# bxlab/bx-python

Hardware: AMD Instinct MI355X
Metric: M overlap-queries/s at 100M x 10M intervals (count-only) (higher is better)
Workload: dtype int32

## Files before the change

### bx-python_amd/csrc/common.hpp

```cpp
#pragma once
#include <hip/hip_runtime.h>

#include <cstdarg>
#include <cstdint>
#include <cstdio>
#include <cstring>
#include <string>

#include "../../include/bxmi.h"

namespace bxmi {

std::string &last_error();
int fail(int code, const char *fmt, ...);

#define BXMI_HIP(expr)                                                                          \
    do {                                                                                        \
        hipError_t _e = (expr);                                                                 \
        if (_e != hipSuccess)                                                                   \
            return ::bxmi::fail(_e == hipErrorOutOfMemory ? BXMI_ENOMEM : BXMI_EHIP, "%s: %s (%s:%d)", #expr, \
                                hipGetErrorString(_e), __FILE__, __LINE__);                     \
    } while (0)

#define BXMI_TRY(expr)            \
// ... 27 lines not shown
        hipError_t e = hipMalloc(&np, want);
        if (e != hipSuccess) return fail(BXMI_ENOMEM, "hipMalloc(%zu): %s", want, hipGetErrorString(e));
        if (keep && p && cap) {
            e = hipMemcpyAsync(np, p, cap, hipMemcpyDeviceToDevice, st);
            if (e == hipSuccess) e = hipStreamSynchronize(st);
            if (e != hipSuccess) {
                (void)hipFree(np);
                return fail(BXMI_EHIP, "grow copy: %s", hipGetErrorString(e));
            }
        }
        if (p) (void)hipFree(p);
        p = np;
        cap = want;
        return BXMI_OK;
    }
    template <typename T>
    T *as() const
    {
        return reinterpret_cast<T *>(p);
    }
};

struct DeviceProps {
    int cus = 256;
    int device = -1;
};
const DeviceProps &device_props();

inline int stream_grid(int64_t work_items, int items_per_block)
{
    int64_t need = (work_items + items_per_block - 1) / items_per_block;
    int64_t cap = (int64_t)device_props().cus * 8;
    int64_t g = need < cap ? need : cap;
    if (g < 1) g = 1;
    return (int)g;
}

inline int64_t div_up(int64_t a, int64_t b) { return (a + b - 1) / b; }

#define BXMI_WAVE 64

#define BX_GLOBAL __attribute__((address_space(1)))
template <typename T>
__device__ __forceinline__ T BX_GLOBAL *as_global(T *p)
{
    return (T BX_GLOBAL *)p;
}
typedef int bx_v4i __attribute__((ext_vector_type(4)));
__device__ __forceinline__ int4 load_int4(const int32_t BX_GLOBAL *p)
{
    const bx_v4i v = *reinterpret_cast<const bx_v4i BX_GLOBAL *>(p);
    return make_int4(v.x, v.y, v.z, v.w);
}
__device__ __forceinline__ void store_int4(int32_t BX_GLOBAL *p, int a, int b, int c, int d)
{
    *reinterpret_cast<bx_v4i BX_GLOBAL *>(p) = bx_v4i{a, b, c, d};
}

__device__ __forceinline__ int lane_id() { return (int)(threadIdx.x & 63); }

#define BXMI_DPP_QUAD_XOR1 0xB1
#define BXMI_DPP_QUAD_XOR2 0x4E
#define BXMI_DPP_HALF_MIRROR 0x141

__device__ __forceinline__ int group8_sum_dpp(int v)
{
    v += __builtin_amdgcn_update_dpp(0, v, BXMI_DPP_QUAD_XOR1, 0xf, 0xf, false);
    v += __builtin_amdgcn_update_dpp(0, v, BXMI_DPP_QUAD_XOR2, 0xf, 0xf, false);
    v += __builtin_amdgcn_update_dpp(0, v, BXMI_DPP_HALF_MIRROR, 0xf, 0xf, false);
    return v;
}

__device__ __forceinline__ int group8_sum_shfl(int v)
{
    v += __shfl_xor(v, 1, 64);
    v += __shfl_xor(v, 2, 64);
    v += __shfl_xor(v, 4, 64);
    return v;
}

__device__ __forceinline__ long long wave_sum_i64(long long v)
{
#pragma unroll
    for (int off = 32; off > 0; off >>= 1) v += __shfl_down(v, off, 64);
    return v;
}

__device__ __forceinline__ unsigned long long lanemask_lt()
{
    return (1ull << lane_id()) - 1ull;
}

__device__ __forceinline__ void block_accumulate_i64(long long v, long long *red, unsigned long long *global_acc)
{
    v = wave_sum_i64(v);
    int w = threadIdx.x >> 6;
    if (lane_id() == 0) red[w] = v;
    __syncthreads();
    if (threadIdx.x == 0) {
        long long s = 0;
        int nw = (blockDim.x + 63) >> 6;
        for (int i = 0; i < nw; i++) s += red[i];
        if (s) atomicAdd(global_acc, (unsigned long long)s);
    }
}

// ... 11 lines not shown
```

### bx-python_amd/csrc/count_bitmap.hpp

```cpp
#pragma once

namespace bxmi {

constexpr int BM_NB = PT_NB;
constexpr unsigned BM_REC_ESC = 0xFFFFFFFFu;
constexpr int BM_MIN_SHIFT = 5;
constexpr int BM_GROUP_TILES = 64;
constexpr int BM_CHUNK = 65536;
constexpr int BM_HARD = 127;
constexpr int BM_LONG_CAP = 480;

struct BmGeom {
    int32_t cmin;
    int32_t cmax;
    int32_t shift;
    int32_t nce;
    int32_t ncs;
    int32_t stride;
    int32_t f;
    int32_t rshift;
    int32_t dshift;
};

__device__ __forceinline__ unsigned bm_len_esc(const BmGeom &g) { return (1u << (32 - g.rshift)) - 1u; }
// ... 159 lines not shown
    return descent;
}

__device__ __forceinline__ void bm_bounds_outer(const int32_t *__restrict__ qs, int64_t nq, const BmBounds &B)
{
    const int first = bm_bounds_upto(B, qs[0]), last = bm_bounds_upto(B, qs[nq - 1]);
    for (int u = 0; u < first; u++) B.bounds[u] = 0u;
    for (int u = last; u <= B.units; u++) B.bounds[u] = (unsigned)nq;
}

template <bool BOUNDS>
__global__ __launch_bounds__(256) void bm_sorted_check_kernel(const int32_t *__restrict__ qs, int64_t nq, unsigned *__restrict__ unsorted, BmBounds B)
{
    if (BOUNDS && blockIdx.x == 0 && threadIdx.x == 0) bm_bounds_outer(qs, nq, B);
    for (int64_t c = blockIdx.x; c * BM_CHECK_CH < nq; c += gridDim.x) {
        if (__hip_atomic_load(unsorted, __ATOMIC_RELAXED, __HIP_MEMORY_SCOPE_WORKGROUP) != 0) return;
        const bool descent = bm_check_chunk<BOUNDS>(qs, nq, c, B);
        if (__syncthreads_or(descent)) {
            if (threadIdx.x == 0) __hip_atomic_store(unsorted, 1u, __ATOMIC_RELAXED, __HIP_MEMORY_SCOPE_WORKGROUP);
            return;
        }
    }
}

__device__ __forceinline__ unsigned bm_bucket_of(int qs, const BmGeom &g)
{
    if (qs < g.cmin) return 0;
    const unsigned b = ((unsigned)qs - (unsigned)g.cmin) >> g.shift;
    return b < (unsigned)(BM_NB - 1) ? b : (unsigned)(BM_NB - 1);
}

template <int SUB>
__device__ __forceinline__ unsigned bm_sort_key_of(int qs, const BmGeom &g)
{
    if (SUB == 1) return bm_bucket_of(qs, g);
    if (qs < g.cmin) return 0;
    const unsigned b = ((unsigned)qs - (unsigned)g.cmin) >> (g.shift - 1);
    return b < (unsigned)(2 * BM_NB - 1) ? b : (unsigned)(2 * BM_NB - 1);
}

__device__ __forceinline__ unsigned bm_record_of(int qs, int qe, const BmGeom &g)
{
    const unsigned rel = (unsigned)qs - (unsigned)g.cmin;
    const unsigned len = (unsigned)qe - (unsigned)qs;
    const bool ok = qs >= g.cmin && (rel >> g.shift) < (unsigned)BM_NB && qe > qs && len < bm_len_esc(g);
    return ok ? ((rel & ((1u << (g.shift + g.f)) - 1u)) | (len << g.rshift)) : BM_REC_ESC;
}

constexpr int BM_PAD_ROOM = 4096 + 544;
#ifndef BM_TS_EXP
#define BM_TS_EXP 0
#endif

template <int THREADS, int ITEMS, bool PAD = false, int SUB = 1, bool TOT = false>
__global__ __launch_bounds__(THREADS) void bm_tile_sort_kernel(const BmSeg *__restrict__ segs, const unsigned short *__restrict__ tile_seg,
                                                               unsigned *__restrict__ recs ,
                                                               unsigned short *__restrict__ slots ,
                                                               unsigned short *__restrict__ tbl ,
                                                               const unsigned *__restrict__ gate ,
                                                               unsigned *__restrict__ tend ,
                                                               unsigned short *__restrict__ tbl2 ,
                                                               const BmSegChunk par, const int npar , const BmParOut po,
                                                               unsigned *__restrict__ tesc = nullptr )
{
    constexpr int TILE = THREADS * ITEMS;
    if (gate && *gate == 0) return;
    static_assert(!TOT || (PAD && SUB == 1), "total-only batches: the persistent walk on padded runs");
    constexpr int NBK = BM_NB * SUB;
    constexpr int BPT = NBK / THREADS;
    static_assert(NBK % THREADS == 0 && (BPT == 2 || BPT == 4), "2 or 4 buckets per thread");
    static_assert(SUB == 1 || (SUB == 2 && !PAD && BPT == 4), "half buckets: packed runs, 1024-thread shapes");
    constexpr int STAGED = PAD ? TILE + 3 * THREADS : TILE;
    constexpr int STRIDE = PAD ? TILE + BM_PAD_ROOM : TILE;
    extern __shared__ __attribute__((aligned(16))) int32_t dyn[];
    unsigned *staged = reinterpret_cast<unsigned *>(dyn);
    unsigned *cnt = staged + STAGED;
    unsigned short *toff = reinterpret_cast<unsigned short *>(cnt + NBK);
    unsigned *scan_tmp = reinterpret_cast<unsigned *>(toff + NBK);
    const int64_t tile = blockIdx.x;
    BmGeom g;
    const int32_t BX_GLOBAL *__restrict__ qs, *__restrict__ qe;
    int64_t nq, ltile, ntiles_seg;
    if (npar) {
        if (blockIdx.x == 0) bm_write_params(par, npar, po);
        int i = 0;
        while (i + 1 < npar && tile >= par.seg[i].tile_end) i++;
        g = par.seg[i].g;
        ltile = tile - par.seg[i].tile0, ntiles_seg = par.seg[i].ntiles;
        qs = as_global(par.seg[i].qs) + ltile * TILE, qe = as_global(par.seg[i].qe) + ltile * TILE;
        nq = par.seg[i].nq - ltile * TILE;
    } else {
        const BmSeg &sg = segs[tile_seg[tile]];
        g = sg.g;
        ltile = tile - sg.tile0, ntiles_seg = sg.ntiles;
        qs = as_global(sg.qs) + ltile * TILE, qe = as_global(sg.qe) + ltile * TILE;
        nq = sg.nq - ltile * TILE;
    }
    if (ltile >= ntiles_seg) return;
    recs += tile * STRIDE, slots += tile * TILE;
    const int64_t base = 0;
    const int n = (int)(nq < TILE ? nq : TILE);
    int n_out = n;
    for (int i = threadIdx.x; i < NBK; i += THREADS) cnt[i] = 0;
    __syncthreads();
    unsigned br[ITEMS];
    int4 vs[ITEMS / 4], ve[ITEMS / 4];
    if (n == TILE) {
#pragma unroll
        for (int j = 0; j < ITEMS / 4; j++) vs[j] = load_int4(qs + base + 4 * (j * THREADS + (int)threadIdx.x));
#pragma unroll
        for (int j = 0; j < ITEMS / 4; j++) ve[j] = load_int4(qe + base + 4 * (j * THREADS + (int)threadIdx.x));
#pragma unroll
        for (int j = 0; j < ITEMS / 4; j++) {
            const unsigned bx = bm_sort_key_of<SUB>(vs[j].x, g), by = bm_sort_key_of<SUB>(vs[j].y, g), bz = bm_sort_key_of<SUB>(vs[j].z, g),
                           bw = bm_sort_key_of<SUB>(vs[j].w, g);
            const unsigned b0 = (unsigned)__builtin_amdgcn_readfirstlane((int)bx);
            if (__all(bx == b0 && by == b0 && bz == b0 && bw == b0)) {
                unsigned r0 = 0;
                if (lane_id() == 0) r0 = atomicAdd(&cnt[b0], 256u);
                r0 = (unsigned)__builtin_amdgcn_readfirstlane((int)r0) + 4u * (unsigned)lane_id();
                br[4 * j + 0] = (b0 << 16) | (r0 + 0);
                br[4 * j + 1] = (b0 << 16) | (r0 + 1);
                br[4 * j + 2] = (b0 << 16) | (r0 + 2);
                br[4 * j + 3] = (b0 << 16) | (r0 + 3);
            } else {
                if (BM_TS_EXP == 1) {
                    const unsigned fake = 4u * (unsigned)(j * THREADS + (int)threadIdx.x);
                    br[4 * j + 0] = (bx << 16) | (fake + 0u), br[4 * j + 1] = (by << 16) | (fake + 1u);
                    br[4 * j + 2] = (bz << 16) | (fake + 2u), br[4 * j + 3] = (bw << 16) | (fake + 3u);
                } else {
                br[4 * j + 0] = (bx << 16) | atomicAdd(&cnt[bx], 1u);
                br[4 * j + 1] = (by << 16) | atomicAdd(&cnt[by], 1u);
                br[4 * j + 2] = (bz << 16) | atomicAdd(&cnt[bz], 1u);
                br[4 * j + 3] = (bw << 16) | atomicAdd(&cnt[bw], 1u);
                }
            }
        }
    } else {
#pragma unroll
        for (int j = 0; j < ITEMS; j++) {
            const int k = j * THREADS + threadIdx.x;
            if (k < n) {
                const unsigned b = bm_sort_key_of<SUB>(qs[base + k], g);
                br[j] = (b << 16) | atomicAdd(&cnt[b], 1u);
            }
        }
    }
    __syncthreads();
    {
        unsigned c[BPT], sum = 0;
#pragma unroll
        for (int u = 0; u < BPT; u++) {
            c[u] = cnt[BPT * threadIdx.x + u];
            sum += c[u];
        }
        unsigned tot;
        unsigned exc;
        if (PAD) {
            const int lane = lane_id();
            const int lanes = (1 << g.f) / BPT;
            unsigned usum = sum;
            for (int d = 1; d < lanes; d <<= 1) usum += (unsigned)__shfl_xor((int)usum, d, 64);
            const unsigned padded = (usum + 3u) & ~3u;
            const bool leader = (lane & (lanes - 1)) == 0;
            const unsigned before = block_exclusive_scan(leader ? padded : 0u, OpSum(), 0u, scan_tmp, &tot);
            const unsigned ubase = (unsigned)__shfl((int)before, lane & ~(lanes - 1), 64);
            unsigned inc = sum;
            for (int d = 1; d < lanes; d <<= 1) {
                const unsigned up = (unsigned)__shfl_up((int)inc, d, 64);
                if ((lane & (lanes - 1)) >= d) inc += up;
            }
            exc = ubase + inc - sum;
            if (leader)
                for (unsigned k = usum; k < padded; k++) staged[ubase + k] = BM_REC_ESC;
            n_out = BM_TS_EXP == 1 ? n : (int)tot;
            if (threadIdx.x == 0) tend[tile] = tot;
        } else {
            exc = block_exclusive_scan(sum, OpSum(), 0u, scan_tmp, &tot);
        }
        unsigned short o[BPT];
#pragma unroll
        for (int u = 0; u < BPT; u++) {
            o[u] = (unsigned short)exc;
            toff[BPT * threadIdx.x + u] = o[u];
            exc += c[u];
        }
        if (SUB == 2) {
            *reinterpret_cast<unsigned *>(tbl + tile * BM_NB + 2 * threadIdx.x) = (unsigned)o[0] | ((unsigned)o[2 % BPT] << 16);
            *reinterpret_cast<uint2 *>(tbl2 + tile * NBK + BPT * threadIdx.x) =
                make_uint2((unsigned)o[0] | ((unsigned)o[1] << 16), (unsigned)o[2 % BPT] | ((unsigned)o[BPT - 1] << 16));
        } else {
        unsigned short *row = tbl + tile * BM_NB + BPT * threadIdx.x;
        if (BPT == 4)
            *reinterpret_cast<uint2 *>(row) = make_uint2((unsigned)o[0] | ((unsigned)o[1] << 16), (unsigned)o[2] | ((unsigned)o[BPT - 1] << 16));
        else
            *reinterpret_cast<unsigned *>(row) = (unsigned)o[0] | ((unsigned)o[1] << 16);
        }
    }
    __syncthreads();
    bool esc = false;
    if (n == TILE) {
        uint2 *l4 = reinterpret_cast<uint2 *>(slots + base);
#pragma unroll
        for (int j = 0; j < ITEMS / 4; j++) {
            const unsigned s0 = toff[br[4 * j + 0] >> 16] + (br[4 * j + 0] & 0xffffu), s1 = toff[br[4 * j + 1] >> 16] + (br[4 * j + 1] & 0xffffu);
            const unsigned s2 = toff[br[4 * j + 2] >> 16] + (br[4 * j + 2] & 0xffffu), s3 = toff[br[4 * j + 3] >> 16] + (br[4 * j + 3] & 0xffffu);
            if (BM_TS_EXP == 3) {
                if ((s0 ^ s1 ^ s2 ^ s3 ^ (unsigned)vs[j].x ^ (unsigned)ve[j].y) == 0x9e3779b9u) staged[0] = s0;
                continue;
            }
            const unsigned r0 = bm_record_of(vs[j].x, ve[j].x, g), r1 = bm_record_of(vs[j].y, ve[j].y, g);
            const unsigned r2 = bm_record_of(vs[j].z, ve[j].z, g), r3 = bm_record_of(vs[j].w, ve[j].w, g);
            staged[s0] = r0, staged[s1] = r1, staged[s2] = r2, staged[s3] = r3;
            if (TOT)
                esc |= r0 == BM_REC_ESC || r1 == BM_REC_ESC || r2 == BM_REC_ESC || r3 == BM_REC_ESC;
            else
                l4[j * THREADS + threadIdx.x] = make_uint2(s0 | (s1 << 16), s2 | (s3 << 16));
        }
    } else {
#pragma unroll
        for (int j = 0; j < ITEMS; j++) {
            const int k = j * THREADS + threadIdx.x;
            if (k < n) {
                const unsigned s = toff[br[j] >> 16] + (br[j] & 0xffffu);
                const unsigned r = bm_record_of(qs[base + k], qe[base + k], g);
                staged[s] = r;
                if (TOT)
                    esc |= r == BM_REC_ESC;
                else
                    slots[base + k] = (unsigned short)s;
            }
        }
    }
    if (TOT) {
        const int any = __syncthreads_or(esc ? 1 : 0);
        if (threadIdx.x == 0) tesc[tile] = (unsigned)(any != 0);
    } else {
        __syncthreads();
    }
    int4 *out = reinterpret_cast<int4 *>(recs + base);
    const int n4 = BM_TS_EXP == 2 ? 0 : (n_out + 3) >> 2;
    for (int i = threadIdx.x; i < n4; i += THREADS) out[i] = reinterpret_cast<const int4 *>(staged)[i];
}


template <int NBK = BM_NB>
__global__ __launch_bounds__(256) void bm_transpose_kernel(const unsigned short *__restrict__ tbl, const BmSeg *__restrict__ segs,
                                                           const unsigned short *__restrict__ tile_seg, int tile_log2,
                                                           unsigned *__restrict__ runT , int64_t ntp,
                                                           unsigned *__restrict__ grpcnt , const unsigned *__restrict__ gate)
{
    __shared__ unsigned short t[BM_GROUP_TILES][66];
    if (gate && *gate == 0) return;
    const int grp = blockIdx.x, b0 = blockIdx.y * 64;
    {
        const int r = threadIdx.x >> 2, q = threadIdx.x & 3;
        const int64_t tile = (int64_t)grp * BM_GROUP_TILES + r;
        const BmSeg &sg = segs[tile_seg[tile]];
        const bool live = tile - sg.tile0 < sg.ntiles;
        const int64_t left = sg.nq - ((tile - sg.tile0) << tile_log2);
        const unsigned ntile = !live ? 0u : (left < ((int64_t)1 << tile_log2) ? (unsigned)left : 1u << tile_log2);
        const unsigned short *row = tbl + tile * NBK + b0 + 16 * q;
        uint4 a = make_uint4(0, 0, 0, 0), c = a;
        if (live) {
            a = *reinterpret_cast<const uint4 *>(row);
            c = *reinterpret_cast<const uint4 *>(row + 8);
        }
        const unsigned w[8] = {a.x, a.y, a.z, a.w, c.x, c.y, c.z, c.w};
#pragma unroll
        for (int i = 0; i < 8; i++) {
            t[r][16 * q + 2 * i] = (unsigned short)(w[i] & 0xffffu);
            t[r][16 * q + 2 * i + 1] = (unsigned short)(w[i] >> 16);
        }
        if (q == 3) t[r][64] = (unsigned short)(b0 + 64 < NBK ? (live ? row[16] : 0) : ntile);
    }
    __syncthreads();
    {
        const int c = threadIdx.x >> 2, q = threadIdx.x & 3;
        unsigned *dst = runT + (int64_t)(b0 + c) * ntp + (int64_t)grp * BM_GROUP_TILES + 16 * q;
        unsigned sum = 0;
        unsigned v[16];
#pragma unroll
        for (int i = 0; i < 16; i++) {
            const unsigned off = t[16 * q + i][c], len = (unsigned)(unsigned short)(t[16 * q + i][c + 1] - t[16 * q + i][c]);
            v[i] = off | (len << 16);
            sum += len;
        }
#pragma unroll
        for (int i = 0; i < 4; i++) reinterpret_cast<uint4 *>(dst)[i] = make_uint4(v[4 * i], v[4 * i + 1], v[4 * i + 2], v[4 * i + 3]);
        sum += __shfl_xor(sum, 1, 64);
        sum += __shfl_xor(sum, 2, 64);
        if (q == 0 && grpcnt) grpcnt[(int64_t)grp * NBK + b0 + c] = sum;
    }
}

constexpr int BM_PLAN_BATCH = 16;
template <bool EMIT, int UNITS>
// ... 363 lines not shown
```

### bx-python_amd/csrc/intervals.hip

```cpp
#include <climits>
#include <vector>
#include <algorithm>
#include <atomic>
#include <condition_variable>
#include <mutex>
#include <thread>
#include <utility>

#include "primitives.hpp"
#include "count_plan.hpp"

#include "count_direct.hpp"
#include "count_parts.hpp"
#include "count_bitmap.hpp"
#include "count_slices.hpp"
#include "find_exchange.hpp"
#include "count_dense.hpp"
#include "find_sorted.hpp"
#include "find_direct.hpp"
#include "find_neighbors.hpp"
#include "cluster.hpp"

namespace bxmi {

static int64_t g_opt_partition = -1;
constexpr int64_t g_opt_partition_min = 4 << 20;
constexpr int PT_MAX_SUB = 1;
constexpr int PT_SLOT_STRIDE = PT_SLOTS + 8;
static int64_t g_opt_sorted_path = 1;
static int64_t g_opt_bitmap = -1;
static int64_t g_opt_bitmap_min = 2 << 20;
static int64_t g_opt_bm_variant = -1;
static int64_t g_opt_fx_direct = -1;
static int64_t g_opt_find_sliced = 1;
static int64_t g_opt_slice = -1;
static int64_t g_opt_sl_f = -1;
constexpr int64_t g_opt_bm_chunk = 0;
static int64_t g_opt_sl_run_cap = 160;
static int64_t g_opt_sl_flat = 1;
constexpr int64_t g_opt_sl_rbits = 20;
static int64_t g_opt_sl_lanes = 0;
static int64_t g_opt_bm_hard_ppm = 2000;
static int64_t g_opt_flat = -1;
static int64_t g_opt_sparse = -1;
static int64_t g_opt_bo_cell_log2 = 0;
constexpr int64_t g_opt_bo_min_per_unit = 4096;
static int64_t g_opt_sorted_cells = 1;
static int64_t g_opt_dense = -1;
static int64_t g_opt_bd_chunk = 0;
static int64_t g_opt_bd_table_from = 0;
static int64_t g_opt_bd_blocks = 0;
static int64_t g_opt_bd_w8 = -1;
static int64_t g_opt_order_skip = -1;
static int64_t g_opt_clumped = -1;
static int64_t g_opt_tot_walk = 1;
static int64_t g_opt_host_chunk = 8 << 20;
static int64_t g_opt_host_touchers = 2;
constexpr int64_t g_opt_bd_unit_log2 = 0;

struct IvlOpt {
    const char *key;
    int64_t *var;
    int64_t (*norm)(int64_t);
};
static const IvlOpt IVL_OPTS[] = {
    {"ivl.partition", &g_opt_partition, nullptr},
    {"ivl.sorted_path", &g_opt_sorted_path, [](int64_t value) -> int64_t { return value != 0; }},
    {"ivl.bitmap_min", &g_opt_bitmap_min, nullptr},
    {"ivl.bitmap", &g_opt_bitmap, nullptr},
    {"ivl.bm_variant", &g_opt_bm_variant, [](int64_t value) -> int64_t { return value < 0 || value > 2 ? -1 : value; }},
    {"ivl.find_sliced", &g_opt_find_sliced, [](int64_t value) -> int64_t { return value != 0; }},
    {"ivl.fx_direct", &g_opt_fx_direct, [](int64_t value) -> int64_t { return value < 0 ? -1 : value != 0; }},
    {"ivl.slice", &g_opt_slice, nullptr},
    {"ivl.sl_f", &g_opt_sl_f, [](int64_t value) -> int64_t { return value > SL_MAX_F ? SL_MAX_F : value; }},
    {"ivl.sl_run_cap", &g_opt_sl_run_cap, [](int64_t value) -> int64_t { return value < 8 ? 8 : value; }},
    {"ivl.sl_flat", &g_opt_sl_flat, [](int64_t value) -> int64_t { return value != 0; }},
    {"ivl.sl_lanes", &g_opt_sl_lanes, [](int64_t value) -> int64_t { return value == 16 || value == 64 ? value : (value == 1 ? -1 : 0);  }},
    {"ivl.bm_hard_ppm", &g_opt_bm_hard_ppm, nullptr},
    {"ivl.flat", &g_opt_flat, nullptr},
    {"ivl.dense", &g_opt_dense, nullptr},
    {"ivl.sparse", &g_opt_sparse, nullptr},
    {"ivl.sorted_cells", &g_opt_sorted_cells, [](int64_t value) -> int64_t { return value != 0; }},
    {"ivl.bo_cell_log2", &g_opt_bo_cell_log2, [](int64_t value) -> int64_t { return value < BO_MIN_K || value > BO_MAX_K ? 0 : value; }},
    {"ivl.bd_chunk", &g_opt_bd_chunk, [](int64_t value) -> int64_t { return value < 0 ? 0 : value; }},
    {"ivl.bd_blocks", &g_opt_bd_blocks, [](int64_t value) -> int64_t { return value != 0; }},
    {"ivl.bd_table_from", &g_opt_bd_table_from, [](int64_t value) -> int64_t { return value < 1 || value > 64 ? 0 : value; }},
    {"ivl.bd_w8", &g_opt_bd_w8, nullptr},
    {"ivl.order_skip", &g_opt_order_skip, nullptr},
    {"ivl.clumped", &g_opt_clumped, nullptr},
    {"ivl.tot_walk", &g_opt_tot_walk, [](int64_t value) -> int64_t { return value != 0; }},
    {"ivl.host_chunk", &g_opt_host_chunk, [](int64_t value) -> int64_t { return value <= 0 ? 0 : ((value + 4095) & ~(int64_t)4095); }},
    {"ivl.host_touchers", &g_opt_host_touchers, [](int64_t value) -> int64_t { return value < 0 ? 0 : (value > 16 ? 16 : value); }},
};
constexpr int IVL_NOPTS = (int)(sizeof(IVL_OPTS) / sizeof(IVL_OPTS[0]));

int ivl_set_option(const char *key, int64_t value)
{
    for (int i = 0; i < IVL_NOPTS; i++)
        if (!strcmp(key, IVL_OPTS[i].key)) {
            *IVL_OPTS[i].var = IVL_OPTS[i].norm ? IVL_OPTS[i].norm(value) : value;
            return 1;
        }
    return 0;
}

int ivl_option_count() { return IVL_NOPTS; }

int ivl_option_at(int i, const char **key, int64_t *value)
{
    if (i < 0 || i >= IVL_NOPTS) return 0;
    *key = IVL_OPTS[i].key;
    *value = *IVL_OPTS[i].var;
    return 1;
}

}

using namespace bxmi;

struct bxmi_ivl {
    std::vector<int32_t> h_start, h_end;
    DevBuf d_start, d_end;
    int64_t n_dev = 0;
// ... 414 lines not shown
    const int64_t nb_used = ((span > 0 ? span : 0) >> g.shift) + 1;
    int f = 0;
    if (g_opt_sl_f >= 0) {
        for (f = (int)g_opt_sl_f; f > 0 && h->sl_need[f] > (unsigned)SL_CAP; f--) {}
    } else {
        for (int k = 1; k <= SL_MAX_F; k++) {
            if (h->sl_need[k] > (unsigned)SL_CAP || g.shift + k > g_opt_sl_rbits || (tile << k) / nb_used > g_opt_sl_run_cap) break;
            f = k;
        }
    }
    g.f = f;
    g.rshift = g.shift + f > 17 ? g.shift + f : 17;
    const int64_t Wu = (int64_t)1 << (g.shift + f);
    int d = 0;
    while (((Wu + SL_MARGIN) >> d) + 1 > SL_DIR_CELLS) d++;
    g.dshift = d;
    g.ncs = (int32_t)((Wu + SL_MARGIN) >> d) + 1;
    g.nce = (int32_t)(Wu >> d) + 1;
    g.stride = 0;
    *lds_bytes = 2 * ((size_t)h->sl_need[f] + 16) + 2 * (size_t)((g.ncs + 2 + 7) & ~7) + 2 * (size_t)(g.nce + 2 + 8);
    *run_len = (tile << f) / nb_used;
    return g;
}

struct BmLaunch {
    const BmSeg *segs;
    const unsigned short *tile_seg;
    bxmi_ivl *owner;
    int64_t ntp;
    int ngroups, tile_log2;
    size_t search_lds;
    const unsigned *gate;
    bool pad = false;
    bool w8 = false;
    bool wide = false;
    bool big = false;
    bool tot = false;
    unsigned long long *tot_slots = nullptr;
    unsigned *descent = nullptr;
    unsigned *xcd_next = nullptr;
    BmSegChunk par;
    int npar = 0;
    BmParOut par_out;
    int n_segs = 1;
    BmGeom g0;
    unsigned long long order_seq = 0;
};

template <int THREADS, int ITEMS>
static int bm_launch_tiles(const BmLaunch &L, hipStream_t st, bool sub = false)
{
    constexpr int TILE = THREADS * ITEMS;
    bxmi_ivl *h = L.owner;
    auto sort = [&](auto kern, int threads, size_t lds, unsigned *tend, unsigned short *tbl2, unsigned *tesc) {
        return launch_lds(kern, dim3((unsigned)L.ntp), dim3(threads), lds, st, L.segs, L.tile_seg, h->bm_recs.as<unsigned>(), h->bm_slots.as<unsigned short>(),
                          h->bm_tbl.as<unsigned short>(), L.gate, tend, tbl2, L.par, L.npar, L.par_out, tesc);
    };
    if (sub) {
        if (THREADS != 1024 || L.pad) return fail(BXMI_ESTATE, "bm_launch_tiles: half buckets need a 1024-thread shape on packed runs");
        constexpr int T2 = THREADS == 1024 ? THREADS : 1024;
        constexpr int I2 = TILE / T2;
        return sort(bm_tile_sort_kernel<T2, I2, false, 2>, T2, (size_t)TILE * 4 + FX_NBK * 4 + FX_NBK * 2 + 64, nullptr, h->fx_tbl2.as<unsigned short>(), nullptr);
    }
    const size_t lds = (size_t)(TILE + (L.pad ? 3 * THREADS : 0)) * 4 + BM_NB * 4 + BM_NB * 2 + 64;
    if (L.pad && L.tot) return sort(bm_tile_sort_kernel<THREADS, ITEMS, true, 1, true>, THREADS, lds, h->bd_tend.as<unsigned>(), nullptr, h->bm_tesc.as<unsigned>());
    if (L.pad) return sort(bm_tile_sort_kernel<THREADS, ITEMS, true>, THREADS, lds, h->bd_tend.as<unsigned>(), nullptr, nullptr);
    return sort(bm_tile_sort_kernel<THREADS, ITEMS, false>, THREADS, lds, nullptr, nullptr, nullptr);
}

template <int THREADS, int ITEMS>
static int bm_launch_unpermute(const BmLaunch &L, unsigned long long *slots, hipStream_t st, const unsigned *cnt = nullptr, unsigned *loff = nullptr,
                               int fx = 0 )
{
    bxmi_ivl *h = L.owner;
    if (!cnt) cnt = h->bm_recs.as<unsigned>();
    const bool find = loff && fx;
    auto unpermute = [&](auto kern) {
        return launch_lds(kern, dim3((unsigned)L.ntp), dim3(THREADS), (size_t)THREADS * ITEMS * sizeof(unsigned), st, cnt, h->bm_slots.as<unsigned short>(), L.segs,
                          L.tile_seg, slots, L.gate, find ? loff : nullptr, find ? h->fx_svq.as<unsigned>() : nullptr,
                          find ? h->fx_parts.as<unsigned long long>() : nullptr, find ? h->fx_tile_tot.as<unsigned long long>() : nullptr);
    };
    if (find && fx == 3) return unpermute(bm_unpermute_kernel<THREADS, ITEMS, 3>);
    if (find) return unpermute(bm_unpermute_kernel<THREADS, ITEMS, 2>);
    return unpermute(bm_unpermute_kernel<THREADS, ITEMS>);
}

#ifndef SL_FIND_U
#define SL_FIND_U 2
#endif
template <int LANES>
static int sl_launch_search(const BmLaunch &L, unsigned grid, hipStream_t st, unsigned *out, unsigned *hc = nullptr)
{
    bxmi_ivl *h = L.owner;
    const bool apart = out != h->bm_recs.as<unsigned>();
    auto search = [&](auto kern) {
        return launch_lds(kern, dim3(grid), dim3(SL_THREADS), L.search_lds, st, L.segs, h->bm_items.as<int4>() + 1, h->bm_items.as<int>(), h->bm_runT.as<unsigned>(),
                          L.ntp, h->bm_recs.as<unsigned>(), apart ? out : nullptr, L.tile_log2, L.gate, apart ? hc : nullptr);
    };
    return apart ? search(sl_search_pipe_kernel<LANES, SL_FIND_U, true>) : search(sl_search_pipe_kernel<LANES, 2, false>);
}

struct BmFindCtx {
    BmLaunch L;
    unsigned sgrid;
    int lanes;
    int variant;
    bool sub = false;
    bool direct = false;
    int f = 0;
// ... 1275 lines not shown
```

Before: 150,200.

## Make bitmap tile sort persistent and prefetch next tile's queries into registers

The tile-sort kernel becomes a persistent grid-stride loop, launched with roughly one workgroup per CU instead of one per tile. Each iteration issues global loads of the next tile's query starts and ends while the current tile is still being scanned, scattered and copied out. Sort keys and records are packed into the already-loaded registers so no extra arrays are needed. The aim is to hide global load latency and cut per-workgroup launch and setup overhead, at the cost of more register pressure, possibly lower occupancy, and more complex uniformity handling.

```diff
diff --git a/bx-python_amd/csrc/common.hpp b/bx-python_amd/csrc/common.hpp
--- a/bx-python_amd/csrc/common.hpp
+++ b/bx-python_amd/csrc/common.hpp
@@ -103,6 +103,10 @@
     const bx_v4i v = *reinterpret_cast<const bx_v4i BX_GLOBAL *>(p);
     return make_int4(v.x, v.y, v.z, v.w);
 }
+__device__ __forceinline__ int4 load_int4_at(const int32_t BX_GLOBAL *p, unsigned bytes)
+{
+    return load_int4(reinterpret_cast<const int32_t BX_GLOBAL *>(reinterpret_cast<const char BX_GLOBAL *>(p) + bytes));
+}
 __device__ __forceinline__ void store_int4(int32_t BX_GLOBAL *p, int a, int b, int c, int d)
 {
     *reinterpret_cast<bx_v4i BX_GLOBAL *>(p) = bx_v4i{a, b, c, d};
diff --git a/bx-python_amd/csrc/count_bitmap.hpp b/bx-python_amd/csrc/count_bitmap.hpp
--- a/bx-python_amd/csrc/count_bitmap.hpp
+++ b/bx-python_amd/csrc/count_bitmap.hpp
@@ -235,6 +235,22 @@
 #define BM_TS_EXP 0
 #endif
 
+__device__ __forceinline__ int64_t bm_uniform(int64_t v)
+{
+    const unsigned lo = (unsigned)__builtin_amdgcn_readfirstlane((int)(unsigned)v), hi = (unsigned)__builtin_amdgcn_readfirstlane((int)(unsigned)((uint64_t)v >> 32));
+    return (int64_t)(((uint64_t)hi << 32) | lo);
+}
+
+__device__ __forceinline__ void bm_into(int &reg, unsigned val) { asm("v_mov_b32 %0, %1" : "+v"(reg) : "v"(val)); }
+__device__ __forceinline__ int &bm_word(int4 &v, int c) { return c == 0 ? v.x : c == 1 ? v.y : c == 2 ? v.z : v.w; }
+
+#ifndef BM_TS_PREFETCH
+#define BM_TS_PREFETCH 1
+#endif
+#ifndef BM_TS_EARLY
+#define BM_TS_EARLY 2
+#endif
+
 template <int THREADS, int ITEMS, bool PAD = false, int SUB = 1, bool TOT = false>
 __global__ __launch_bounds__(THREADS) void bm_tile_sort_kernel(const BmSeg *__restrict__ segs, const unsigned short *__restrict__ tile_seg,
                                                                unsigned *__restrict__ recs ,
@@ -244,7 +260,8 @@
                                                                unsigned *__restrict__ tend ,
                                                                unsigned short *__restrict__ tbl2 ,
                                                                const BmSegChunk par, const int npar , const BmParOut po,
-                                                               unsigned *__restrict__ tesc = nullptr )
+                                                               unsigned *__restrict__ tesc ,
+                                                               const int64_t ntp )
 {
     constexpr int TILE = THREADS * ITEMS;
     if (gate && *gate == 0) return;
@@ -255,177 +272,234 @@
     static_assert(SUB == 1 || (SUB == 2 && !PAD && BPT == 4), "half buckets: packed runs, 1024-thread shapes");
     constexpr int STAGED = PAD ? TILE + 3 * THREADS : TILE;
     constexpr int STRIDE = PAD ? TILE + BM_PAD_ROOM : TILE;
+    constexpr int EARLY = BM_TS_EARLY < ITEMS / 4 ? BM_TS_EARLY : ITEMS / 4;
+    constexpr int NST = ITEMS / 4 + (PAD ? 1 : 0);
+    constexpr int NOBODY = STRIDE / 4 - 1;
+    static_assert(STAGED % 4 == 0 && STRIDE % 4 == 0 && NST * THREADS * 4 >= STAGED && NST * THREADS * 4 <= STAGED + NBK, "copy-out: whole tile, inside the LDS");
+    static_assert(!PAD || (NOBODY >= STAGED / 4 && NST * THREADS * 4 <= STRIDE), "copy-out: inside the tile's stride");
     extern __shared__ __attribute__((aligned(16))) int32_t dyn[];
     unsigned *staged = reinterpret_cast<unsigned *>(dyn);
     unsigned *cnt = staged + STAGED;
     unsigned short *toff = reinterpret_cast<unsigned short *>(cnt + NBK);
     unsigned *scan_tmp = reinterpret_cast<unsigned *>(toff + NBK);
-    const int64_t tile = blockIdx.x;
-    BmGeom g;
-    const int32_t BX_GLOBAL *__restrict__ qs, *__restrict__ qe;
-    int64_t nq, ltile, ntiles_seg;
-    if (npar) {
-        if (blockIdx.x == 0) bm_write_params(par, npar, po);
-        int i = 0;
-        while (i + 1 < npar && tile >= par.seg[i].tile_end) i++;
-        g = par.seg[i].g;
-        ltile = tile - par.seg[i].tile0, ntiles_seg = par.seg[i].ntiles;
-        qs = as_global(par.seg[i].qs) + ltile * TILE, qe = as_global(par.seg[i].qe) + ltile * TILE;
-        nq = par.seg[i].nq - ltile * TILE;
-    } else {
-        const BmSeg &sg = segs[tile_seg[tile]];
-        g = sg.g;
-        ltile = tile - sg.tile0, ntiles_seg = sg.ntiles;
-        qs = as_global(sg.qs) + ltile * TILE, qe = as_global(sg.qe) + ltile * TILE;
-        nq = sg.nq - ltile * TILE;
-    }
-    if (ltile >= ntiles_seg) return;
-    recs += tile * STRIDE, slots += tile * TILE;
-    const int64_t base = 0;
-    const int n = (int)(nq < TILE ? nq : TILE);
-    int n_out = n;
+    if (npar && blockIdx.x == 0) bm_write_params(par, npar, po);
+    auto uniform_ref = [](BmTileRef r) {
+        r.seg = __builtin_amdgcn_readfirstlane(r.seg), r.n = __builtin_amdgcn_readfirstlane(r.n), r.ltile = bm_uniform(r.ltile);
+        return r;
+    };
+    auto ref_of = [&](int64_t t) { return npar ? uniform_ref(bm_tile_ref(par.seg, npar, nullptr, t, TILE)) : uniform_ref(bm_tile_ref(segs, 0, tile_seg, t, TILE)); };
+    auto uniform_queries = [](const BmSeg &sg, int64_t ltile, const int32_t BX_GLOBAL *&s, const int32_t BX_GLOBAL *&e) {
+        s = (const int32_t BX_GLOBAL *)bm_uniform((int64_t)(as_global(sg.qs) + ltile * TILE));
+        e = (const int32_t BX_GLOBAL *)bm_uniform((int64_t)(as_global(sg.qe) + ltile * TILE));
+    };
+    auto queries_of = [&](const BmTileRef &r, const int32_t BX_GLOBAL *&s, const int32_t BX_GLOBAL *&e) {
+        if (npar)
+            uniform_queries(par.seg[r.seg], r.ltile, s, e);
+        else
+            uniform_queries(segs[r.seg], r.ltile, s, e);
+    };
+    auto uniform_geom = [](const BmGeom &m) {
+        BmGeom g = m;
+        g.cmin = __builtin_amdgcn_readfirstlane(m.cmin), g.shift = __builtin_amdgcn_readfirstlane(m.shift);
+        g.f = __builtin_amdgcn_readfirstlane(m.f), g.rshift = __builtin_amdgcn_readfirstlane(m.rshift);
+        return g;
+    };
     for (int i = threadIdx.x; i < NBK; i += THREADS) cnt[i] = 0;
     __syncthreads();
-    unsigned br[ITEMS];
     int4 vs[ITEMS / 4], ve[ITEMS / 4];
-    if (n == TILE) {
-#pragma unroll
-        for (int j = 0; j < ITEMS / 4; j++) vs[j] = load_int4(qs + base + 4 * (j * THREADS + (int)threadIdx.x));
-#pragma unroll
-        for (int j = 0; j < ITEMS / 4; j++) ve[j] = load_int4(qe + base + 4 * (j * THREADS + (int)threadIdx.x));
-#pragma unroll
-        for (int j = 0; j < ITEMS / 4; j++) {
-            const unsigned bx = bm_sort_key_of<SUB>(vs[j].x, g), by = bm_sort_key_of<SUB>(vs[j].y, g), bz = bm_sort_key_of<SUB>(vs[j].z, g),
-                           bw = bm_sort_key_of<SUB>(vs[j].w, g);
-            const unsigned b0 = (unsigned)__builtin_amdgcn_readfirstlane((int)bx);
-            if (__all(bx == b0 && by == b0 && bz == b0 && bw == b0)) {
-                unsigned r0 = 0;
-                if (lane_id() == 0) r0 = atomicAdd(&cnt[b0], 256u);
-                r0 = (unsigned)__builtin_amdgcn_readfirstlane((int)r0) + 4u * (unsigned)lane_id();
-                br[4 * j + 0] = (b0 << 16) | (r0 + 0);
-                br[4 * j + 1] = (b0 << 16) | (r0 + 1);
-                br[4 * j + 2] = (b0 << 16) | (r0 + 2);
-                br[4 * j + 3] = (b0 << 16) | (r0 + 3);
+    unsigned bre[EARLY > 0 ? 4 * EARLY : 1];
+    const int64_t step = gridDim.x;
+    BmTileRef cur = ref_of(blockIdx.x);
+    bool have = false;
+    for (int64_t tile = blockIdx.x; tile < ntp; tile += step) {
+        unsigned tid = threadIdx.x;
+        asm volatile("" : "+v"(tid));
+        const unsigned lane16 = 16u * tid;
+        const int64_t tile_next = tile + step;
+        BmTileRef nxt;
+        nxt.seg = 0, nxt.ltile = 0, nxt.n = 0;
+        if (tile_next < ntp) nxt = ref_of(tile_next);
+        const bool ask = BM_TS_PREFETCH && nxt.n == TILE && cur.n > 0;
+        const int32_t BX_GLOBAL *nqs = nullptr, *nqe = nullptr;
+        if (ask) queries_of(nxt, nqs, nqe);
+        if (cur.n > 0) {
+            const BmGeom g = npar ? uniform_geom(par.seg[cur.seg].g) : uniform_geom(segs[cur.seg].g);
+            const int32_t BX_GLOBAL *qs, *qe;
+            queries_of(cur, qs, qe);
+            unsigned *const rout = recs + tile * STRIDE;
+            unsigned short *const sout = slots + tile * TILE;
+            const int n = cur.n;
+            int n_out = n;
+            bool esc = false;
+            if (n == TILE) {
+                if (!have) {
+#pragma unroll
+                    for (int j = 0; j < ITEMS / 4; j++) vs[j] = load_int4_at(qs, lane16 + (unsigned)(j * 16 * THREADS));
+#pragma unroll
+                    for (int j = 0; j < ITEMS / 4; j++) ve[j] = load_int4_at(qe, lane16 + (unsigned)(j * 16 * THREADS));
+                }
+#pragma unroll
+                for (int j = 0; j < ITEMS / 4; j++) {
+                    const unsigned bx = bm_sort_key_of<SUB>(vs[j].x, g), by = bm_sort_key_of<SUB>(vs[j].y, g), bz = bm_sort_key_of<SUB>(vs[j].z, g),
+                                   bw = bm_sort_key_of<SUB>(vs[j].w, g);
+                    const unsigned b0 = (unsigned)__builtin_amdgcn_readfirstlane((int)bx);
+                    unsigned k0, k1, k2, k3;
+                    if (__all(bx == b0 && by == b0 && bz == b0 && bw == b0)) {
+                        unsigned r0 = 0;
+                        if (lane_id() == 0) r0 = atomicAdd(&cnt[b0], 256u);
+                        r0 = (unsigned)__builtin_amdgcn_readfirstlane((int)r0) + 4u * (unsigned)lane_id();
+                        k0 = (b0 << 16) | (r0 + 0), k1 = (b0 << 16) | (r0 + 1), k2 = (b0 << 16) | (r0 + 2), k3 = (b0 << 16) | (r0 + 3);
+                    } else if (BM_TS_EXP == 1) {
+                        const unsigned fake = 4u * (unsigned)(j * THREADS + (int)tid);
+                        k0 = (bx << 16) | (fake + 0u), k1 = (by << 16) | (fake + 1u), k2 = (bz << 16) | (fake + 2u), k3 = (bw << 16) | (fake + 3u);
+                    } else {
+                        k0 = (bx << 16) | atomicAdd(&cnt[bx], 1u);
+                        k1 = (by << 16) | atomicAdd(&cnt[by], 1u);
+                        k2 = (bz << 16) | atomicAdd(&cnt[bz], 1u);
+                        k3 = (bw << 16) | atomicAdd(&cnt[bw], 1u);
+                    }
+                    const unsigned r0 = bm_record_of(vs[j].x, ve[j].x, g), r1 = bm_record_of(vs[j].y, ve[j].y, g);
+                    const unsigned r2 = bm_record_of(vs[j].z, ve[j].z, g), r3 = bm_record_of(vs[j].w, ve[j].w, g);
+                    if (TOT) esc |= r0 == BM_REC_ESC || r1 == BM_REC_ESC || r2 == BM_REC_ESC || r3 == BM_REC_ESC;
+                    if (j < EARLY)
+                        bre[(4 * j + 0) % (4 * EARLY + !EARLY)] = k0, bre[(4 * j + 1) % (4 * EARLY + !EARLY)] = k1, bre[(4 * j + 2) % (4 * EARLY + !EARLY)] = k2,
+                                                          bre[(4 * j + 3) % (4 * EARLY + !EARLY)] = k3;
+                    else
+                        bm_into(vs[j].x, k0), bm_into(vs[j].y, k1), bm_into(vs[j].z, k2), bm_into(vs[j].w, k3);
+                    bm_into(ve[j].x, r0), bm_into(ve[j].y, r1), bm_into(ve[j].z, r2), bm_into(ve[j].w, r3);
+                }
             } else {
-                if (BM_TS_EXP == 1) {
-                    const unsigned fake = 4u * (unsigned)(j * THREADS + (int)threadIdx.x);
-                    br[4 * j + 0] = (bx << 16) | (fake + 0u), br[4 * j + 1] = (by << 16) | (fake + 1u);
-                    br[4 * j + 2] = (bz << 16) | (fake + 2u), br[4 * j + 3] = (bw << 16) | (fake + 3u);
+#pragma unroll
+                for (int j = 0; j < ITEMS; j++) {
+                    const int k = j * THREADS + tid;
+                    if (k < n) {
+                        const unsigned b = bm_sort_key_of<SUB>(qs[k], g);
+                        bm_word(ve[j / 4], j % 4) = (int)((b << 16) | atomicAdd(&cnt[b], 1u));
+                    }
+                }
+            }
+            __syncthreads();
+            if (ask) {
+#pragma unroll
+                for (int j = 0; j < EARLY; j++) vs[j] = load_int4_at(nqs, lane16 + (unsigned)(j * 16 * THREADS));
+            } else {
+#pragma unroll
+                for (int j = 0; j < EARLY; j++) vs[j] = make_int4(0, 0, 0, 0);
+            }
+            {
+                unsigned c[BPT], sum = 0;
+#pragma unroll
+                for (int u = 0; u < BPT; u++) {
+                    c[u] = cnt[BPT * tid + u];
+                    cnt[BPT * tid + u] = 0;
+                    sum += c[u];
+                }
+                unsigned tot;
+                unsigned exc;
+                if (PAD) {
+                    const int lane = lane_id();
+                    const int lanes = (1 << g.f) / BPT;
+                    unsigned usum = sum;
+                    for (int d = 1; d < lanes; d <<= 1) usum += (unsigned)__shfl_xor((int)usum, d, 64);
+                    const unsigned padded = (usum + 3u) & ~3u;
+                    const bool leader = (lane & (lanes - 1)) == 0;
+                    const unsigned before = block_exclusive_scan(leader ? padded : 0u, OpSum(), 0u, scan_tmp, &tot);
+                    const unsigned ubase = (unsigned)__shfl((int)before, lane & ~(lanes - 1), 64);
+                    unsigned inc = sum;
+                    for (int d = 1; d < lanes; d <<= 1) {
+                        const unsigned up = (unsigned)__shfl_up((int)inc, d, 64);
+                        if ((lane & (lanes - 1)) >= d) inc += up;
+                    }
+                    exc = ubase + inc - sum;
+                    if (leader)
+                        for (unsigned k = usum; k < padded; k++) staged[ubase + k] = BM_REC_ESC;
+                    n_out = BM_TS_EXP == 1 ? n : (int)tot;
+                    if (tid == 0) tend[tile] = tot;
                 } else {
-                br[4 * j + 0] = (bx << 16) | atomicAdd(&cnt[bx], 1u);
-                br[4 * j + 1] = (by << 16) | atomicAdd(&cnt[by], 1u);
-                br[4 * j + 2] = (bz << 16) | atomicAdd(&cnt[bz], 1u);
-                br[4 * j + 3] = (bw << 16) | atomicAdd(&cnt[bw], 1u);
+                    exc = block_exclusive_scan(sum, OpSum(), 0u, scan_tmp, &tot);
                 }
-            }
-        }
-    } else {
-#pragma unroll
-        for (int j = 0; j < ITEMS; j++) {
-            const int k = j * THREADS + threadIdx.x;
-            if (k < n) {
-                const unsigned b = bm_sort_key_of<SUB>(qs[base + k], g);
-                br[j] = (b << 16) | atomicAdd(&cnt[b], 1u);
-            }
-        }
-    }
-    __syncthreads();
-    {
-        unsigned c[BPT], sum = 0;
-#pragma unroll
-        for (int u = 0; u < BPT; u++) {
-            c[u] = cnt[BPT * threadIdx.x + u];
-            sum += c[u];
-        }
-        unsigned tot;
-        unsigned exc;
-        if (PAD) {
-            const int lane = lane_id();
-            const int lanes = (1 << g.f) / BPT;
-            unsigned usum = sum;
-            for (int d = 1; d < lanes; d <<= 1) usum += (unsigned)__shfl_xor((int)usum, d, 64);
-            const unsigned padded = (usum + 3u) & ~3u;
-            const bool leader = (lane & (lanes - 1)) == 0;
-            const unsigned before = block_exclusive_scan(leader ? padded : 0u, OpSum(), 0u, scan_tmp, &tot);
-            const unsigned ubase = (unsigned)__shfl((int)before, lane & ~(lanes - 1), 64);
-            unsigned inc = sum;
-            for (int d = 1; d < lanes; d <<= 1) {
-                const unsigned up = (unsigned)__shfl_up((int)inc, d, 64);
-                if ((lane & (lanes - 1)) >= d) inc += up;
-            }
-            exc = ubase + inc - sum;
-            if (leader)
-                for (unsigned k = usum; k < padded; k++) staged[ubase + k] = BM_REC_ESC;
-            n_out = BM_TS_EXP == 1 ? n : (int)tot;
-            if (threadIdx.x == 0) tend[tile] = tot;
-        } else {
-            exc = block_exclusive_scan(sum, OpSum(), 0u, scan_tmp, &tot);
-        }
-        unsigned short o[BPT];
-#pragma unroll
-        for (int u = 0; u < BPT; u++) {
-            o[u] = (unsigned short)exc;
-            toff[BPT * threadIdx.x + u] = o[u];
-            exc += c[u];
-        }
-        if (SUB == 2) {
-            *reinterpret_cast<unsigned *>(tbl + tile * BM_NB + 2 * threadIdx.x) = (unsigned)o[0] | ((unsigned)o[2 % BPT] << 16);
-            *reinterpret_cast<uint2 *>(tbl2 + tile * NBK + BPT * threadIdx.x) =
-                make_uint2((unsigned)o[0] | ((unsigned)o[1] << 16), (unsigned)o[2 % BPT] | ((unsigned)o[BPT - 1] << 16));
-        } else {
-        unsigned short *row = tbl + tile * BM_NB + BPT * threadIdx.x;
-        if (BPT == 4)
-            *reinterpret_cast<uint2 *>(row) = make_uint2((unsigned)o[0] | ((unsigned)o[1] << 16), (unsigned)o[2] | ((unsigned)o[BPT - 1] << 16));
-        else
-            *reinterpret_cast<unsigned *>(row) = (unsigned)o[0] | ((unsigned)o[1] << 16);
-        }
-    }
-    __syncthreads();
-    bool esc = false;
-    if (n == TILE) {
-        uint2 *l4 = reinterpret_cast<uint2 *>(slots + base);
-#pragma unroll
-        for (int j = 0; j < ITEMS / 4; j++) {
-            const unsigned s0 = toff[br[4 * j + 0] >> 16] + (br[4 * j + 0] & 0xffffu), s1 = toff[br[4 * j + 1] >> 16] + (br[4 * j + 1] & 0xffffu);
-            const unsigned s2 = toff[br[4 * j + 2] >> 16] + (br[4 * j + 2] & 0xffffu), s3 = toff[br[4 * j + 3] >> 16] + (br[4 * j + 3] & 0xffffu);
-            if (BM_TS_EXP == 3) {
-                if ((s0 ^ s1 ^ s2 ^ s3 ^ (unsigned)vs[j].x ^ (unsigned)ve[j].y) == 0x9e3779b9u) staged[0] = s0;
-                continue;
-            }
-            const unsigned r0 = bm_record_of(vs[j].x, ve[j].x, g), r1 = bm_record_of(vs[j].y, ve[j].y, g);
-            const unsigned r2 = bm_record_of(vs[j].z, ve[j].z, g), r3 = bm_record_of(vs[j].w, ve[j].w, g);
-            staged[s0] = r0, staged[s1] = r1, staged[s2] = r2, staged[s3] = r3;
-            if (TOT)
-                esc |= r0 == BM_REC_ESC || r1 == BM_REC_ESC || r2 == BM_REC_ESC || r3 == BM_REC_ESC;
-            else
-                l4[j * THREADS + threadIdx.x] = make_uint2(s0 | (s1 << 16), s2 | (s3 << 16));
-        }
-    } else {
-#pragma unroll
-        for (int j = 0; j < ITEMS; j++) {
-            const int k = j * THREADS + threadIdx.x;
-            if (k < n) {
-                const unsigned s = toff[br[j] >> 16] + (br[j] & 0xffffu);
-                const unsigned r = bm_record_of(qs[base + k], qe[base + k], g);
-                staged[s] = r;
-                if (TOT)
-                    esc |= r == BM_REC_ESC;
-                else
-                    slots[base + k] = (unsigned short)s;
-            }
-        }
-    }
-    if (TOT) {
-        const int any = __syncthreads_or(esc ? 1 : 0);
-        if (threadIdx.x == 0) tesc[tile] = (unsigned)(any != 0);
-    } else {
-        __syncthreads();
-    }
-    int4 *out = reinterpret_cast<int4 *>(recs + base);
-    const int n4 = BM_TS_EXP == 2 ? 0 : (n_out + 3) >> 2;
-    for (int i = threadIdx.x; i < n4; i += THREADS) out[i] = reinterpret_cast<const int4 *>(staged)[i];
-}
-
+                unsigned short o[BPT];
+#pragma unroll
+                for (int u = 0; u < BPT; u++) {
+                    o[u] = (unsigned short)exc;
+                    toff[BPT * tid + u] = o[u];
+                    exc += c[u];
+                }
+                if (SUB == 2) {
+                    *reinterpret_cast<unsigned *>(tbl + tile * BM_NB + 2 * tid) = (unsigned)o[0] | ((unsigned)o[2 % BPT] << 16);
+                    *reinterpret_cast<uint2 *>(tbl2 + tile * NBK + BPT * tid) =
+                        make_uint2((unsigned)o[0] | ((unsigned)o[1] << 16), (unsigned)o[2 % BPT] | ((unsigned)o[BPT - 1] << 16));
+                } else {
+                    unsigned short *row = tbl + tile * BM_NB + BPT * tid;
+                    if (BPT == 4)
+                        *reinterpret_cast<uint2 *>(row) = make_uint2((unsigned)o[0] | ((unsigned)o[1] << 16), (unsigned)o[2] | ((unsigned)o[BPT - 1] << 16));
+                    else
+                        *reinterpret_cast<unsigned *>(row) = (unsigned)o[0] | ((unsigned)o[1] << 16);
+                }
+            }
+            __syncthreads();
+            if (n == TILE) {
+                char *const l4 = reinterpret_cast<char *>(sout);
+#pragma unroll
+                for (int j = 0; j < ITEMS / 4; j++) {
+                    const unsigned k0 = j < EARLY ? bre[(4 * j + 0) % (4 * EARLY + !EARLY)] : (unsigned)vs[j].x, k1 = j < EARLY ? bre[(4 * j + 1) % (4 * EARLY + !EARLY)] : (unsigned)vs[j].y;
+                    const unsigned k2 = j < EARLY ? bre[(4 * j + 2) % (4 * EARLY + !EARLY)] : (unsigned)vs[j].z, k3 = j < EARLY ? bre[(4 * j + 3) % (4 * EARLY + !EARLY)] : (unsigned)vs[j].w;
+                    const unsigned s0 = toff[k0 >> 16] + (k0 & 0xffffu), s1 = toff[k1 >> 16] + (k1 & 0xffffu);
+                    const unsigned s2 = toff[k2 >> 16] + (k2 & 0xffffu), s3 = toff[k3 >> 16] + (k3 & 0xffffu);
+                    if (BM_TS_EXP == 3) {
+                        if ((s0 ^ s1 ^ s2 ^ s3 ^ (unsigned)(ve[j].x ^ ve[j].y ^ ve[j].z ^ ve[j].w)) == 0x9e3779b9u) staged[0] = s0;
+                        continue;
+                    }
+                    staged[s0] = (unsigned)ve[j].x, staged[s1] = (unsigned)ve[j].y, staged[s2] = (unsigned)ve[j].z, staged[s3] = (unsigned)ve[j].w;
+                        if (!TOT) *reinterpret_cast<uint2 *>(l4 + (8u * tid + (unsigned)(j * 8 * THREADS))) = make_uint2(s0 | (s1 << 16), s2 | (s3 << 16));
+                }
+            } else {
+#pragma unroll
+                for (int j = 0; j < ITEMS; j++) {
+                    const int k = j * THREADS + tid;
+                    if (k < n) {
+                        const unsigned kj = (unsigned)bm_word(ve[j / 4], j % 4);
+                        const unsigned s = toff[kj >> 16] + (kj & 0xffffu);
+                        const unsigned r = bm_record_of(qs[k], qe[k], g);
+                        staged[s] = r;
+                        if (TOT)
+                            esc |= r == BM_REC_ESC;
+                        else
+                            sout[k] = (unsigned short)s;
+                    }
+                }
+            }
+            if (TOT) {
+                const int any = __syncthreads_or(esc ? 1 : 0);
+                if (tid == 0) tesc[tile] = (unsigned)(any != 0);
+            } else {
+                __syncthreads();
+            }
+            if (ask) {
+#pragma unroll
+                for (int j = EARLY; j < ITEMS / 4; j++) vs[j] = load_int4_at(nqs, lane16 + (unsigned)(j * 16 * THREADS));
+#pragma unroll
+                for (int j = 0; j < ITEMS / 4; j++) ve[j] = load_int4_at(nqe, lane16 + (unsigned)(j * 16 * THREADS));
+            } else {
+#pragma unroll
+                for (int j = EARLY; j < ITEMS / 4; j++) vs[j] = make_int4(0, 0, 0, 0);
+#pragma unroll
+                for (int j = 0; j < ITEMS / 4; j++) ve[j] = make_int4(0, 0, 0, 0);
+            }
+            char *const out = reinterpret_cast<char *>(rout);
+            const int n4 = (n_out + 3) >> 2;
+            if (BM_TS_EXP != 2) {
+#pragma unroll
+                for (int j = 0; j < NST; j++) {
+                    const unsigned i = (unsigned)j * THREADS + tid;
+                    *reinterpret_cast<int4 *>(out + 16u * (PAD && i >= (unsigned)n4 ? (unsigned)NOBODY : i)) = reinterpret_cast<const int4 *>(staged)[i];
+                }
+            }
+        }
+        cur = nxt;
+        have = ask;
+    }
+}
 
 template <int NBK = BM_NB>
 __global__ __launch_bounds__(256) void bm_transpose_kernel(const unsigned short *__restrict__ tbl, const BmSeg *__restrict__ segs,
diff --git a/bx-python_amd/csrc/intervals.hip b/bx-python_amd/csrc/intervals.hip
--- a/bx-python_amd/csrc/intervals.hip
+++ b/bx-python_amd/csrc/intervals.hip
@@ -9,6 +9,7 @@
 
 #include "primitives.hpp"
 #include "count_plan.hpp"
+#include "tile_loop.hpp"
 
 #include "count_direct.hpp"
 #include "count_parts.hpp"
@@ -31,6 +32,7 @@
 static int64_t g_opt_bitmap = -1;
 static int64_t g_opt_bitmap_min = 2 << 20;
 static int64_t g_opt_bm_variant = -1;
+static int64_t g_opt_ts_groups = 0;
 static int64_t g_opt_fx_direct = -1;
 static int64_t g_opt_find_sliced = 1;
 static int64_t g_opt_slice = -1;
@@ -69,6 +71,7 @@
     {"ivl.bitmap_min", &g_opt_bitmap_min, nullptr},
     {"ivl.bitmap", &g_opt_bitmap, nullptr},
     {"ivl.bm_variant", &g_opt_bm_variant, [](int64_t value) -> int64_t { return value < 0 || value > 2 ? -1 : value; }},
+    {"ivl.ts_groups", &g_opt_ts_groups, [](int64_t value) -> int64_t { return value < 0 ? 0 : value; }},
     {"ivl.find_sliced", &g_opt_find_sliced, [](int64_t value) -> int64_t { return value != 0; }},
     {"ivl.fx_direct", &g_opt_fx_direct, [](int64_t value) -> int64_t { return value < 0 ? -1 : value != 0; }},
     {"ivl.slice", &g_opt_slice, nullptr},
@@ -589,9 +592,10 @@
 {
     constexpr int TILE = THREADS * ITEMS;
     bxmi_ivl *h = L.owner;
+    const unsigned groups = (unsigned)bm_loop_groups(L.ntp, device_props().cus, g_opt_ts_groups);
     auto sort = [&](auto kern, int threads, size_t lds, unsigned *tend, unsigned short *tbl2, unsigned *tesc) {
-        return launch_lds(kern, dim3((unsigned)L.ntp), dim3(threads), lds, st, L.segs, L.tile_seg, h->bm_recs.as<unsigned>(), h->bm_slots.as<unsigned short>(),
-                          h->bm_tbl.as<unsigned short>(), L.gate, tend, tbl2, L.par, L.npar, L.par_out, tesc);
+        return launch_lds(kern, dim3(groups), dim3(threads), lds, st, L.segs, L.tile_seg, h->bm_recs.as<unsigned>(), h->bm_slots.as<unsigned short>(),
+                          h->bm_tbl.as<unsigned short>(), L.gate, tend, tbl2, L.par, L.npar, L.par_out, tesc, L.ntp);
     };
     if (sub) {
         if (THREADS != 1024 || L.pad) return fail(BXMI_ESTATE, "bm_launch_tiles: half buckets need a 1024-thread shape on packed runs");
diff --git a/bx-python_amd/csrc/tile_loop.hpp b/bx-python_amd/csrc/tile_loop.hpp
--- /dev/null
+++ b/bx-python_amd/csrc/tile_loop.hpp
@@ -0,0 +1,41 @@
+#pragma once
+#include <cstdint>
+#if defined(__HIPCC__)
+#define BT_HD __host__ __device__ __forceinline__
+#else
+#define BT_HD inline
+#endif
+
+namespace bxmi {
+
+struct BmTileRef {
+    int seg;
+    int64_t ltile;
+    int n;
+};
+
+template <typename Seg>
+BT_HD BmTileRef bm_tile_ref(const Seg *seg, int npar, const unsigned short *tile_seg, int64_t tile, int tile_size)
+{
+    int i = 0;
+    if (npar)
+        while (i + 1 < npar && tile >= seg[i].tile_end) i++;
+    else
+        i = (int)((reinterpret_cast<const uint32_t *>(tile_seg)[tile >> 1] >> (16 * (int)(tile & 1))) & 0xffffu);
+    BmTileRef r;
+    r.seg = i;
+    r.ltile = tile - seg[i].tile0;
+    const int64_t left = seg[i].nq - r.ltile * tile_size;
+    r.n = r.ltile < 0 || r.ltile >= seg[i].ntiles || left <= 0 ? 0 : (int)(left < tile_size ? left : tile_size);
+    return r;
+}
+
+BT_HD int64_t bm_loop_groups(int64_t ntp, int64_t cus, int64_t opt)
+{
+    const int64_t g = opt > 0 ? opt : cus;
+    return g < ntp ? (g < 1 ? 1 : g) : ntp;
+}
+
+BT_HD int64_t bm_loop_trips(int64_t ntp, int64_t groups, int64_t wg) { return wg < ntp ? (ntp - wg + groups - 1) / groups : 0; }
+
+}
```

After: 151,600, median of 6. About the same (+1.0%).
